# Peiyannn/MM-PDE

Hardware: AMD Instinct MI355X
Metric: MM-PDE rollout node-updates/sec, cylinder 2521-node mesh, 1/2/4/8 GPUs (higher is better)
Workload: dtype f32 (every GNN GEMM fp32-emulated by the fp16x3 split with fp32 accumulate: edge message_net_2, node update_net_1/_2 and message_net_1 projections, embedding; DMM, ItpNet, res_cut, kNN and heads exact fp32); 1 GPU; cy-mmpde; trajectories_per_gpu=16, global_trajectories=16, nodes_per_trajectory=2521, neighbors=35, parallelism=trajectory-shard x1 (no data-path collective), rollout=autoregressive (pred -> next input), launch=eager, three HIP streams, stream_priorities=False

## Files before the change

### mm-pde_amd/csrc/layer.hip

```cpp
#include "common.hpp"
#include <type_traits>
#include "f16x3.hpp"
#include "layer.hpp"

namespace {

constexpr int LH = 128;
constexpr int ET = 16;
constexpr int ESL = 4;
constexpr int ERING = 3;
constexpr int EPF = ERING - 1;
constexpr int SLOT4 = 512;
constexpr int NLDA = LH + 4;

__device__ __forceinline__ void tile_schedule(int bid, int G, int ntiles, int &first, int &stride,
                                              int &count) {
    const int x = bid & 7, i = bid >> 3;
    const int q = G >> 3, rem = G & 7;
    const int nW = q + (x < rem ? 1 : 0);
    const int cum = x * q + min(x, rem);
    const int lo = (int)((int64_t)ntiles * cum / G);
    const int hi = (int)((int64_t)ntiles * (cum + nW) / G);
    first = lo + i;
    stride = nW;
// ... 319 lines not shown
                        for (int cc = 0; cc < CT; ++cc) Ssave[cc] = S[cc];
                        pend = cC.j;
                    }
#pragma unroll
                    for (int cc = 0; cc < CT; ++cc) S[cc] = (f32x4){0.0f, 0.0f, 0.0f, 0.0f};
                }
                cC.next(rpt);
                slot = slot == ERING - 1 ? 0 : slot + 1;
            }
            __syncthreads();
        }
        finish_pending();
    }
}

struct NodeArgs {
    const float *h, *mean;
    int64_t n;
    const float *u1, *c1;
    int64_t ld_u1;
    const float *u2, *c2;
    const float *bn_w, *bn_b, *bn_rm, *bn_rv;
    float eps;
    float *h_out;
    const float *w1n, *b1n;
    int64_t ld_w1n;
    float *a_out, *b_out;
    const float *u, *pos;
    mmpde_gnn_scales sc;
    const char *pk, *pkn;
    float *rmx_out;
    int64_t seg_n;
    const int32_t *div_deg = nullptr;
    int div_k = 0;
    EdgeSplit split;
};

constexpr int NLD = 132;
constexpr int RB = 2;
constexpr int ROWS = 16 * RB;
constexpr int NODE_WPE = 4;

__device__ __forceinline__ void prep_item(int idx, int &row, int &part) {
    row = (idx >> 6) * 8 + (idx & 7);
    part = (idx >> 3) & 7;
}

__device__ __forceinline__ void prep_fetch(const float *src, int64_t lds, int64_t row0, int64_t nrows_valid,
                                           bool global, int row, int part, float4 (&x)[4]) {
    const int64_t srow = global ? min(row0 + row, nrows_valid - 1) : row;
    const float *sp = src + srow * lds + 16 * part;
#pragma unroll
    for (int q = 0; q < 4; ++q) x[q] = *(const float4 *)(sp + 4 * q);
}

template <bool F16X3>
__device__ __forceinline__ void prep_finish(float4 (&x)[4], int64_t srow, int row, int part, float4 *img,
                                            int KT, int kofs, float *rs, float *copy, const int32_t *div_deg,
                                            int div_k, const EdgeSplit *split) {
    if (split && split->units > 0) {
        const SideUnits su = side_units(*split, srow);
        for (int64_t w = su.lo; w <= su.hi; ++w) {
            const float *q4 = split->side + ((su.sg * split->units + w) * 16 + (su.q & 15)) * 128 + 16 * part;
#pragma unroll
            for (int q = 0; q < 4; ++q) {
                const float4 y = *(const float4 *)(q4 + 4 * q);
                x[q] = make_float4(x[q].x + y.x, x[q].y + y.y, x[q].z + y.z, x[q].w + y.w);
            }
        }
    }
    if (div_k > 0) {
        const float d = div_deg ? (float)max(div_deg[srow], 1) : (float)div_k;
        div_rows_rn(x, d);
    }
    if (copy) {
#pragma unroll
        for (int q = 0; q < 4; ++q) *(float4 *)(copy + row * NLD + 16 * part + 4 * q) = x[q];
    }
    const int rb = row >> 4, rr = row & 15;
    if (F16X3) {
        float m = 0.0f;
#pragma unroll
        for (int q = 0; q < 4; ++q) m = absmax4(m, x[q]);
        m = absmax_stride8(m);
        const float s = split_scale(m);
        if (part == 0) rs[row] = s;
#pragma unroll
        for (int q = 0; q < 4; ++q) x[q] = make_float4(x[q].x * s, x[q].y * s, x[q].z * s, x[q].w * s);
        const int KS = KT / 32;
        const int ks = (kofs + 16 * part) >> 5;
        const int g0 = 2 * (part & 1);
#pragma unroll
        for (int hh = 0; hh < 2; ++hh) {
            half8 hi, lo;
            split8_rn(x[2 * hh], x[2 * hh + 1], hi, lo);
            float4 *d = img + ((rb * KS + ks) * 2) * 64 + 16 * (g0 + hh) + rr;
            d[0] = *(const float4 *)&hi;
            d[64] = *(const float4 *)&lo;
        }
    } else {
        const int KJ = KT / 16;
        const int j = (kofs >> 4) + part;
#pragma unroll
        for (int q = 0; q < 4; ++q) img[(rb * KJ + j) * 64 + 16 * q + rr] = x[q];
    }
}

template <bool F16X3>
__device__ __forceinline__ void prep(const float *src, int64_t lds, int64_t row0, int64_t nrows_valid,
                                     bool global, float4 *img, int KT, int kofs, float *rs,
                                     float *copy = nullptr, int t0 = -1, int nthr = 512,
                                     const int32_t *div_deg = nullptr, int div_k = 0,
                                     const EdgeSplit *split = nullptr) {
    for (int idx = t0 < 0 ? (int)threadIdx.x : (int)threadIdx.x - t0; idx < ROWS * 8; idx += nthr) {
        int row, part;
        prep_item(idx, row, part);
        float4 x[4];
        prep_fetch(src, lds, row0, nrows_valid, global, row, part, x);
        const int64_t srow = global ? min(row0 + row, nrows_valid - 1) : row;
        prep_finish<F16X3>(x, srow, row, part, img, KT, kofs, rs, copy, div_deg, div_k, split);
    }
}

template <bool F16X3, int NS>
struct BOps {
    half8 h[F16X3 ? NS : 1], l[F16X3 ? NS : 1];
    float4 w[F16X3 ? 1 : NS];
    __device__ __forceinline__ void load(const char *bimg, int KSB, int ct, int sb0,
                                         const float *wrow, int wk0, int lane) {
#pragma unroll
        for (int s = 0; s < NS; ++s) {
            if (F16X3) {
                h[s] = bfrag(bimg, KSB, ct, sb0 + s, 0, lane);
                l[s] = bfrag(bimg, KSB, ct, sb0 + s, 1, lane);
            } else {
                w[s] = *(const float4 *)(wrow + wk0 + 16 * s + 4 * (lane >> 4));
            }
        }
    }
};

template <bool F16X3, int NS>
__device__ __forceinline__ void gemm_tile(f32x4 *acc, const float4 *img, int KT, int s0,
                                          const BOps<F16X3, NS> &B, int lane) {
#pragma unroll
    for (int s = 0; s < NS; ++s) {
#pragma unroll
        for (int rb = 0; rb < RB; ++rb) {
            if (F16X3) {
                const int KS = KT / 32;
                const float4 h4 = img[((rb * KS + s0 + s) * 2) * 64 + lane];
                const float4 l4 = img[((rb * KS + s0 + s) * 2 + 1) * 64 + lane];
                const half8 ah = *(const half8 *)&h4, al = *(const half8 *)&l4;
                acc[rb] = mfma_f16(ah, B.h[s], acc[rb]);
                acc[rb] = mfma_f16(ah, B.l[s], acc[rb]);
                acc[rb] = mfma_f16(al, B.h[s], acc[rb]);
            } else {
                const int KJ = KT / 16;
                const float4 a = img[(rb * KJ + s0 + s) * 64 + lane];
                acc[rb] = mfma16(a.x, B.w[s].x, acc[rb]);
                acc[rb] = mfma16(a.y, B.w[s].y, acc[rb]);
                acc[rb] = mfma16(a.z, B.w[s].z, acc[rb]);
                acc[rb] = mfma16(a.w, B.w[s].w, acc[rb]);
            }
        }
    }
}

constexpr int MAX_TW = 16;

struct RowValues {
    float t = 0.0f, x = 0.0f, y = 0.0f, u[MAX_TW];
    __device__ __forceinline__ void fetch(const mmpde_gnn_scales &sc, const float *pos, const float *uu,
                                          int64_t row, int tw) {
        const float *pr = sc.pos_xy ? pos + row * 2 : pos + row * 3 + 1;
        x = pr[0];
        y = pr[1];
        t = sc.pos_xy ? (sc.t_ptr ? *sc.t_ptr : sc.t) : pr[-1];
#pragma unroll
        for (int c = 0; c < MAX_TW; ++c) u[c] = c < tw ? uu[row * tw + c] : 0.0f;
    }
    __device__ __forceinline__ void store(float (*rowv)[ROWS], const mmpde_gnn_scales &sc, int tid, int tw) const {
        rowv[0][tid] = t * sc.inv_tmax;
        rowv[1][tid] = x * sc.inv_lx;
        rowv[2][tid] = y * sc.inv_ly;
#pragma unroll
        for (int c = 0; c < MAX_TW; ++c)
            if (c < tw) rowv[3 + c][tid] = u[c];
    }
};

struct W1C {
    float du = 0.0f, dx = 0.0f, dy = 0.0f, t = 0.0f, b = 0.0f, isa = 1.0f, isb = 1.0f;
    template <bool F16X3>
    __device__ __forceinline__ void load(const float *w1r, const float *b1, const char *pk, int col,
                                         int tw) {
        du = w1r[256];
        dx = w1r[256 + tw];
        dy = w1r[257 + tw];
        t = w1r[258 + tw];
        b = b1[col];
        if (F16X3) {
            const float *su = (const float *)(pk + kPkW1 + 131072);
            isa = pow2_inv(su[col]);
            isb = pow2_inv(su[128 + col]);
        }
    }
};

template <bool F16X3>
__device__ __forceinline__ void proj_phase(const BOps<F16X3, F16X3 ? 4 : 8> &bA, const float4 *img,
                                           const float *rs, const float *rowv, const W1C &w,
                                           const char *pk, const float *w1r, int tw, int64_t row0,
                                           int64_t n, int64_t seg_n, float *a_out, float *b_out,
                                           float *rmx_out, uint32_t *arrived, int wave, int lane) {
    constexpr int S1 = F16X3 ? 4 : 8;
    const int col = 16 * wave + (lane & 15), g = lane >> 4;
    f32x4 aA[RB], aB[RB];
#pragma unroll
    for (int rb = 0; rb < RB; ++rb) aA[rb] = aB[rb] = (f32x4){0.0f, 0.0f, 0.0f, 0.0f};
    uint32_t amx[RB][4], bmx[RB][4];
#pragma unroll
    for (int rb = 0; rb < RB; ++rb)
#pragma unroll
        for (int q = 0; q < 4; ++q) amx[rb][q] = bmx[rb][q] = 0u;
    const bool full = row0 + ROWS <= n;
    float *ap = a_out + (row0 + 4 * g) * LH + col, *bp = b_out + (row0 + 4 * g) * LH + col;
    auto node_term = [&](int lr) {
        float node = w.du * rowv[3 * ROWS + lr];
        for (int c = 1; c < tw; ++c) node += w1r[256 + c] * rowv[(3 + c) * ROWS + lr];
        return node + w.dx * rowv[ROWS + lr] + w.dy * rowv[2 * ROWS + lr];
    };
    gemm_tile<F16X3, S1>(aA, img, 128, 0, bA, lane);
    {
        BOps<F16X3, S1> bB;
        bB.load(pk + kPkW1, 4, 8 + wave, 0, w1r, 128, lane);
        gemm_tile<F16X3, S1>(aB, img, 128, 0, bB, lane);
#pragma unroll
        for (int rb = 0; rb < RB; ++rb) {
#pragma unroll
            for (int q = 0; q < 4; ++q) {
                const int lr = 16 * rb + 4 * g + q;
                if (full || row0 + lr < n) {
                    float za = aA[rb][q], zb = aB[rb][q];
                    if (F16X3) {
                        const float ir = pow2_inv(rs[lr]);
                        za = za * ir * w.isa;
                        zb = zb * ir * w.isb;
                    }
                    const float node = node_term(lr);
                    const float va = za + node + w.t * rowv[lr] + w.b;
                    const float vb = zb - node;
                    ap[(16 * rb + q) * LH] = va;
                    bp[(16 * rb + q) * LH] = vb;
                    amx[rb][q] = __builtin_bit_cast(uint32_t, fmaxf(fabsf(va), 0.0f));
                    bmx[rb][q] = __builtin_bit_cast(uint32_t, fmaxf(fabsf(vb), 0.0f));
                }
            }
        }
    }
    if (rmx_out) {
        __shared__ uint32_t red[8][ROWS][2];
#pragma unroll
        for (int rb = 0; rb < RB; ++rb) {
#pragma unroll
            for (int q = 0; q < 4; ++q) {
                uint32_t ua = amx[rb][q], ub = bmx[rb][q];
                ua = max(ua, dpp_u<0xB1>(ua));
                ub = max(ub, dpp_u<0xB1>(ub));
                ua = max(ua, dpp_u<0x4E>(ua));
                ub = max(ub, dpp_u<0x4E>(ub));
                ua = max(ua, dpp_u<0x141>(ua));
                ub = max(ub, dpp_u<0x141>(ub));
                ua = max(ua, dpp_u<0x140>(ua));
                ub = max(ub, dpp_u<0x140>(ub));
                if ((lane & 15) == 0) {
                    red[wave][16 * rb + 4 * g + q][0] = ua;
                    red[wave][16 * rb + 4 * g + q][1] = ub;
                }
            }
        }
        asm volatile("s_waitcnt lgkmcnt(0)" ::: "memory");
        uint32_t prev = 0;
        if (lane == 0) prev = __hip_atomic_fetch_add(arrived, 1u, __ATOMIC_RELAXED, __HIP_MEMORY_SCOPE_WORKGROUP);
        prev = __builtin_amdgcn_readfirstlane(prev);
        asm volatile("s_waitcnt lgkmcnt(0)" ::: "memory");
        if (prev == 7) {
            static_assert(2 * ROWS % 64 == 0, "row maxima: whole waves");
#pragma unroll
            for (int l0 = 0; l0 < 2 * ROWS; l0 += 64) {
                const int l = l0 + lane, row = l >> 1, e = l & 1;
                uint32_t m = red[0][row][e];
#pragma unroll
                for (int w2 = 1; w2 < 8; ++w2) m = max(m, red[w2][row][e]);
                const int64_t grow = row0 + row, b0 = row0 + 16 * (row >> 4);
                const bool live = grow < n;
                if (live) rmx_out[2 * grow + e] = __builtin_bit_cast(float, m);
                const bool part1 = grow >= (b0 / seg_n + 1) * seg_n;
                uint32_t mx0 = live && !part1 ? m : 0u, mx1 = live && part1 ? m : 0u;
                uint32_t mn0 = live && !part1 ? m : 0x7f800000u, mn1 = live && part1 ? m : 0x7f800000u;
                auto xmax = [&](uint32_t &v, auto O) {
                    v = max(v, __builtin_bit_cast(uint32_t, xor_lane_f<decltype(O)::value>(__builtin_bit_cast(float, v))));
                };
                auto xmin = [&](uint32_t &v, auto O) {
                    v = min(v, __builtin_bit_cast(uint32_t, xor_lane_f<decltype(O)::value>(__builtin_bit_cast(float, v))));
                };
                using X2 = std::integral_constant<int, 2>;
                using X4 = std::integral_constant<int, 4>;
                using X8 = std::integral_constant<int, 8>;
                using X16 = std::integral_constant<int, 16>;
                xmax(mx0, X2{}); xmax(mx1, X2{}); xmin(mn0, X2{}); xmin(mn1, X2{});
                xmax(mx0, X4{}); xmax(mx1, X4{}); xmin(mn0, X4{}); xmin(mn1, X4{});
                xmax(mx0, X8{}); xmax(mx1, X8{}); xmin(mn0, X8{}); xmin(mn1, X8{});
                xmax(mx0, X16{}); xmax(mx1, X16{}); xmin(mn0, X16{}); xmin(mn1, X16{});
                if ((l & 31) < 2 && b0 < n) {
                    float *rec = rmx_out + row_max_floats(n) + 8 * (b0 / 16);
                    rec[e] = __builtin_bit_cast(float, mx0);
                    rec[2 + e] = __builtin_bit_cast(float, mn0);
                    rec[4 + e] = __builtin_bit_cast(float, mx1);
                    rec[6 + e] = __builtin_bit_cast(float, mn1);
                }
            }
        }
    }
}

#ifdef MMPDE_NODE_STAMPS
__device__ uint64_t *g_node_stamps;
#define NODE_STAMP(i)                                                                       \
    do {                                                                                   \
        if (threadIdx.x == 0) g_node_stamps[(int64_t)blockIdx.x * 8 + (i)] = __builtin_amdgcn_s_memrealtime(); \
    } while (0)
#else
#define NODE_STAMP(i) \
    do {              \
    } while (0)
#endif

template <bool NEXT, bool F16X3>
__global__ __launch_bounds__(512, NODE_WPE) void gnn_node_kernel(NodeArgs p) {
    NODE_STAMP(0);
    __shared__ float4 img[RB * 16 * 64];
    __shared__ float stage[ROWS * NLD];
    __shared__ float hres[ROWS * NLD];
    __shared__ float rs[4][ROWS];
    __shared__ float rowv[3 + MAX_TW][ROWS];
    __shared__ uint32_t rng_arrived;
    const int tid = threadIdx.x, wave = tid >> 6, lane = tid & 63;
    const int r = lane & 15, g = lane >> 4;
    const int col = 16 * wave + r;
    if (tid == 0) rng_arrived = 0;
    const int tw = p.sc.tw > 1 ? p.sc.tw : 1;
    constexpr int S1 = F16X3 ? 4 : 8;
    const float *wu1 = p.u1 + (int64_t)col * p.ld_u1, *wu2 = p.u2 + (int64_t)col * LH;
    const int64_t row0 = (int64_t)blockIdx.x * ROWS;
    RowValues rv;
    if (tid < ROWS) rv.fetch(p.sc, p.pos, p.u, min(row0 + tid, p.n - 1), tw);
    const float u1_wt = wu1[256], u1_b = p.c1[col];
    const float u1_is = F16X3 ? pow2_inv(((const float *)(p.pk + kPkU1 + 131072))[col]) : 1.0f;
    const float u2_b = p.c2[col];
    BnAffine bn;
    bn.set(p.bn_rm[col], p.bn_rv[col], p.bn_w[col], p.bn_b[col], p.eps);
    const float u2_is = F16X3 ? pow2_inv(((const float *)(p.pk + kPkU2 + 65536))[col]) : 1.0f;
    const float *w1r = NEXT ? p.w1n + (int64_t)col * p.ld_w1n : nullptr;
    W1C w1c;
    if (NEXT) w1c.load<F16X3>(w1r, p.b1n, p.pkn, col, tw);
    BOps<F16X3, S1> bH, bM, bU2;
    bH.load(p.pk + kPkU1, 8, wave, 0, wu1, 0, lane);
    if (tid < ROWS) rv.store(rowv, p.sc, tid, tw);

    NODE_STAMP(1);
    if (tid < 256) prep<F16X3>(p.h, LH, row0, p.n, true, img, 256, 0, rs[0], hres, 0, 256);
    else prep<F16X3>(p.mean, LH, row0, p.n, true, img, 256, 128, rs[1], nullptr, 256, 256, p.div_deg,
                     p.div_k, &p.split);
    __syncthreads();
    NODE_STAMP(2);

    {
        f32x4 aH[RB], aM[RB];
#pragma unroll
        for (int rb = 0; rb < RB; ++rb) aH[rb] = aM[rb] = (f32x4){0.0f, 0.0f, 0.0f, 0.0f};
        gemm_tile<F16X3, S1>(aH, img, 256, 0, bH, lane);
        bM.load(p.pk + kPkU1, 8, wave, S1, wu1, 128, lane);
        gemm_tile<F16X3, S1>(F16X3 ? aM : aH, img, 256, S1, bM, lane);
        bU2.load(p.pk + kPkU2, 4, wave, 0, wu2, 0, lane);
#pragma unroll
        for (int rb = 0; rb < RB; ++rb) {
#pragma unroll
            for (int q = 0; q < 4; ++q) {
                const int lr = 16 * rb + 4 * g + q;
                float v = aH[rb][q];
                if (F16X3) v = v * pow2_inv(rs[0][lr]) * u1_is + aM[rb][q] * pow2_inv(rs[1][lr]) * u1_is;
                stage[lr * NLD + col] = fmaxf(v + u1_wt * rowv[0][lr] + u1_b, 0.0f);
            }
        }
    }
    NODE_STAMP(3);
    __syncthreads();
    prep<F16X3>(stage, NLD, 0, ROWS, false, img, 128, 0, rs[2]);
    __syncthreads();
    NODE_STAMP(4);

    BOps<F16X3, S1> bA;
    {
        f32x4 acc[RB];
#pragma unroll
        for (int rb = 0; rb < RB; ++rb) acc[rb] = (f32x4){0.0f, 0.0f, 0.0f, 0.0f};
        gemm_tile<F16X3, S1>(acc, img, 128, 0, bU2, lane);
        if (NEXT) bA.load(p.pkn + kPkW1, 4, wave, 0, w1r, 0, lane);
        const bool full = row0 + ROWS <= p.n;
        float *hp = p.h_out + (row0 + 4 * g) * LH + col;
#pragma unroll
        for (int rb = 0; rb < RB; ++rb) {
#pragma unroll
            for (int q = 0; q < 4; ++q) {
                const int lr = 16 * rb + 4 * g + q;
                float z = acc[rb][q];
                if (F16X3) z = z * pow2_inv(rs[2][lr]) * u2_is;
                const float x = hres[lr * NLD + col] + fmaxf(z + u2_b, 0.0f);
                const float y = bn(x);
                if (full || row0 + lr < p.n) hp[(16 * rb + q) * LH] = y;
                if (NEXT) stage[lr * NLD + col] = y;
            }
        }
    }
    NODE_STAMP(5);
    if constexpr (NEXT) {
        __syncthreads();
        prep<F16X3>(stage, NLD, 0, ROWS, false, img, 128, 0, rs[3]);
        __syncthreads();
        NODE_STAMP(6);
        proj_phase<F16X3>(bA, img, rs[3], &rowv[0][0], w1c, p.pkn, w1r, tw, row0, p.n, p.seg_n,
                              p.a_out, p.b_out, p.rmx_out, &rng_arrived, wave, lane);
    }
    NODE_STAMP(7);
}

struct EmbedArgs {
    const float *u, *pos;
    int64_t n;
    mmpde_gnn_scales sc;
    mmpde_gnn_embed_params e;
    float *h_out;
    const float *w1, *b1;
    int64_t ld_w1;
    float *a_out, *b_out;
    const char *pk;
    float *rmx_out;
    int64_t seg_n;
};

template <bool F16X3>
__global__ __launch_bounds__(512, NODE_WPE) void gnn_embed_kernel(EmbedArgs p) {
    constexpr int S1 = F16X3 ? 4 : 8;
    __shared__ float4 img[RB * 8 * 64];
    __shared__ float stage[ROWS * NLD];
    __shared__ float rs[ROWS];
    __shared__ uint32_t rng_arrived;
    __shared__ float rsz[ROWS];
    __shared__ float rowv[3 + MAX_TW][ROWS];
    const int tid = threadIdx.x, wave = tid >> 6, lane = tid & 63;
    const int g = lane >> 4;
    const int64_t row0 = (int64_t)blockIdx.x * ROWS;
    const int col = 16 * wave + (lane & 15);
    const int tw = p.sc.tw > 1 ? p.sc.tw : 1;
    if (tid == 0) rng_arrived = 0;
    RowValues rv;
    if (tid < ROWS) rv.fetch(p.sc, p.pos, p.u, min(row0 + tid, p.n - 1), tw);
    const mmpde_gnn_embed_params &e = p.e;
    BOps<false, 8> b3;
    BOps<true, 4> b3h;
    float w3_is = 1.0f;
    if (F16X3) {
        const float *wr = e.w3 + (int64_t)col * LH;
        float4 w[8];
#pragma unroll
        for (int s = 0; s < 4; ++s) {
            w[2 * s] = *(const float4 *)(wr + 32 * s + 8 * g);
            w[2 * s + 1] = *(const float4 *)(wr + 32 * s + 8 * g + 4);
        }
        float m = 0.0f;
#pragma unroll
        for (int i = 0; i < 8; ++i) m = absmax4(m, w[i]);
        m = fmaxf(m, __shfl_xor(m, 16, 64));
        m = fmaxf(m, __shfl_xor(m, 32, 64));
        const float sw = split_scale(m);
        w3_is = pow2_inv(sw);
#pragma unroll
        for (int i = 0; i < 8; ++i) w[i] = make_float4(w[i].x * sw, w[i].y * sw, w[i].z * sw, w[i].w * sw);
#pragma unroll
        for (int s = 0; s < 4; ++s) split8_rn(w[2 * s], w[2 * s + 1], b3h.h[s], b3h.l[s]);
    } else {
        b3.load(nullptr, 0, 0, 0, e.w3 + (int64_t)col * LH, 0, lane);
    }
    const float h_b = e.b3[col];
    BnAffine bn4;
    bn4.set(e.bn4_rm[col], e.bn4_rv[col], e.bn4_w[col], e.bn4_b[col], e.eps);
    const float *w1r = p.w1 + (int64_t)col * p.ld_w1;
    W1C w1c;
    w1c.load<F16X3>(w1r, p.b1, p.pk, col, tw);
    const int c = tid & 127;
    const float *zwr = e.w0 + (int64_t)c * (tw + 3);
    const float zw0 = zwr[0], zw1 = zwr[tw], zw2 = zwr[tw + 1], zw3 = zwr[tw + 2];
    const float zb = e.b0[c];
    BnAffine bn1;
    bn1.set(e.bn1_rm[c], e.bn1_rv[c], e.bn1_w[c], e.bn1_b[c], e.eps);
    if (tid < ROWS) rv.store(rowv, p.sc, tid, tw);
    __syncthreads();
    for (int row = tid >> 7; row < ROWS; row += 4) {
        float v = zb + zw0 * rowv[3][row];
        for (int ch = 1; ch < tw; ++ch) v += zwr[ch] * rowv[3 + ch][row];
        v = v + zw1 * rowv[1][row] + zw2 * rowv[2][row] + zw3 * rowv[0][row];
        stage[row * NLD + c] = fmaxf(bn1(v), 0.0f);
    }
    __syncthreads();
    prep<F16X3>(stage, NLD, 0, ROWS, false, img, 128, 0, rsz);
    __syncthreads();
    BOps<F16X3, S1> bA;
    {
        f32x4 acc[RB];
#pragma unroll
        for (int rb = 0; rb < RB; ++rb) acc[rb] = (f32x4){0.0f, 0.0f, 0.0f, 0.0f};
        if (F16X3) {
            gemm_tile<true, 4>(acc, img, 128, 0, b3h, lane);
#pragma unroll
            for (int rb = 0; rb < RB; ++rb)
#pragma unroll
                for (int q = 0; q < 4; ++q) acc[rb][q] *= pow2_inv(rsz[16 * rb + 4 * g + q]) * w3_is;
        } else {
            gemm_tile<false, 8>(acc, img, 128, 0, b3, lane);
        }
        bA.load(p.pk + kPkW1, 4, wave, 0, w1r, 0, lane);
        const bool full = row0 + ROWS <= p.n;
        float *hp = p.h_out + (row0 + 4 * g) * LH + col;
#pragma unroll
        for (int rb = 0; rb < RB; ++rb) {
#pragma unroll
            for (int q = 0; q < 4; ++q) {
                const int lr = 16 * rb + 4 * g + q;
                const float y = bn4(acc[rb][q] + h_b);
                if (full || row0 + lr < p.n) hp[(16 * rb + q) * LH] = y;
                stage[lr * NLD + col] = y;
            }
        }
    }
    __syncthreads();
    prep<F16X3>(stage, NLD, 0, ROWS, false, img, 128, 0, rs);
    __syncthreads();
    proj_phase<F16X3>(bA, img, rs, &rowv[0][0], w1c, p.pk, w1r, tw, row0, p.n, p.seg_n,
                          p.a_out, p.b_out, p.rmx_out, &rng_arrived, wave, lane);
}

inline bool al16(const void *q) { return ((uintptr_t)q & 15u) == 0; }

int device_cus() {
    int dev = 0, cus = 0;
    if (hipGetDevice(&dev) != hipSuccess) return 256;
    if (hipDeviceGetAttribute(&cus, hipDeviceAttributeMultiprocessorCount, dev) != hipSuccess || cus < 1)
        return 256;
    return cus;
}

}

int launch_edge_stage(const float *a, const float *b, const int32_t *nbr, const int32_t *deg,
                      int64_t n, int k, int64_t seg_n, const mmpde_gnn_layer_params *p, const char *pk,
                      const float *rmx, float *mean, float *side, int64_t side_cap,
                      EdgeSplit *split, hipStream_t st, uint32_t *relu_mask, bool rng) {
    if (split) *split = EdgeSplit{};
    MMPDE_REQUIRE(!relu_mask || (!pk && al16(relu_mask)));
    MMPDE_REQUIRE(a && b && nbr && p && mean && n > 0 && k > 0 && n <= (int64_t)INT32_MAX);
    MMPDE_REQUIRE(al16(a) && al16(b) && al16(p->msg2_w) && al16(mean));
    MMPDE_REQUIRE(!pk || (rmx && al16(pk) && al16(rmx)));
    const int64_t ntiles = (n + ET - 1) / ET;
    MMPDE_REQUIRE(ntiles * ((k + ESL - 1) / ESL) < (int64_t)INT32_MAX);
    const int cus = device_cus();
    if (pk)
        return launch_edge_wave(a, b, nbr, deg, n, k, seg_n, p->msg2_b, pk, rmx, rng, mean, side, side_cap, cus,
                                split, st);
    EdgeArgs e{a, b, nbr, n, k, (int)ntiles, p->msg2_w, p->msg2_b, nullptr, nullptr, mean, deg, relu_mask};
    const int grid = ntiles < cus ? (int)ntiles : cus;
    if (deg) hipLaunchKernelGGL((gnn_edge_kernel<false, true>), dim3(grid), dim3(768), 0, st, e);
    else hipLaunchKernelGGL((gnn_edge_kernel<false, false>), dim3(grid), dim3(768), 0, st, e);
    MMPDE_RET_LAUNCH();
    return MMPDE_OK;
}

__global__ __launch_bounds__(256) void row_max_kernel(const float *__restrict__ a, const float *__restrict__ b,
                                                      int64_t n, float *__restrict__ rmx) {
    const int64_t row = (int64_t)blockIdx.x * 8 + (threadIdx.x >> 5);
    const int c4 = threadIdx.x & 31;
    const int64_t rr = min(row, n - 1);
    float ma = absmax4(0.0f, *(const float4 *)(a + rr * LH + 4 * c4));
    float mb = absmax4(0.0f, *(const float4 *)(b + rr * LH + 4 * c4));
#pragma unroll
    for (int o = 16; o >= 1; o >>= 1) {
        ma = fmaxf(ma, __shfl_xor(ma, o, 32));
        mb = fmaxf(mb, __shfl_xor(mb, o, 32));
    }
    if (c4 == 0 && row < n) *(float2 *)(rmx + 2 * row) = make_float2(ma, mb);
}

__global__ __launch_bounds__(256) void row_scale_kernel(const float *__restrict__ rmx, const int32_t *__restrict__ nbr,
                                                        const int32_t *__restrict__ deg, int64_t n, int k,
                                                        float *__restrict__ rsc) {
    const int64_t row = (int64_t)blockIdx.x * 256 + threadIdx.x;
    if (row >= n) return;
    const int kk = deg ? max(min(deg[row], k), 1) : k;
    const float mb = nbr_bmax<36>(rmx, nbr + row * k, kk, (uint32_t)(n - 1));
    rsc[row] = row_split_scale(rmx[2 * row] + mb);
}

__global__ __launch_bounds__(256) void edge_finish_kernel(float *__restrict__ mean, EdgeSplit sp,
                                                          const int32_t *__restrict__ deg, int64_t n) {
    const int64_t row = (int64_t)blockIdx.x * 32 + (threadIdx.x >> 3);
    const int part = threadIdx.x & 7;
    if (row >= n) return;
    float *mp = mean + row * LH + 16 * part;
    float4 x[4];
#pragma unroll
    for (int q = 0; q < 4; ++q) x[q] = *(const float4 *)(mp + 4 * q);
    const SideUnits su = side_units(sp, row);
    for (int64_t w = su.lo; w <= su.hi; ++w) {
        const float *q4 = sp.side + ((su.sg * sp.units + w) * 16 + (su.q & 15)) * LH + 16 * part;
#pragma unroll
        for (int q = 0; q < 4; ++q) {
            const float4 y = *(const float4 *)(q4 + 4 * q);
            x[q] = make_float4(x[q].x + y.x, x[q].y + y.y, x[q].z + y.z, x[q].w + y.w);
        }
    }
    div_rows_rn(x, deg ? (float)max(deg[row], 1) : (float)sp.k);
#pragma unroll
    for (int q = 0; q < 4; ++q) *(float4 *)(mp + 4 * q) = x[q];
}

int64_t edge_mean_f16x3_ws_bytes(int64_t n) {
    const int64_t tail = ((n + 15) / 16) * 16 * LH;
    return kLayerPack + (row_max_floats(n) + tail) * 4;
}

int launch_edge_mean_f16x3(const float *a, const float *b, const int32_t *nbr, const int32_t *deg, int64_t n,
                           int k, const float *w2, const float *b2, float *mean, uint32_t *relu_mask, void *ws,
                           hipStream_t st) {
    MMPDE_REQUIRE(a && b && nbr && w2 && b2 && mean && ws && n > 0 && k > 0 && n <= (int64_t)INT32_MAX);
    MMPDE_REQUIRE(al16(a) && al16(b) && al16(w2) && al16(mean) && al16(ws));
    MMPDE_REQUIRE(!relu_mask || al16(relu_mask));
    const int64_t ntiles = (n + ET - 1) / ET;
    MMPDE_REQUIRE(ntiles * ((k + ESL - 1) / ESL) < (int64_t)INT32_MAX);
    char *pk = (char *)ws;
    float *rmx = (float *)(pk + kLayerPack);
    float *rsc = rmx + row_max_floats(n);
    PackSrc src{};
    src.w[0] = w2;
    src.ld[0] = LH;
    hipLaunchKernelGGL(pack_f16x3_kernel<128>, dim3(128, 1), dim3(128), 0, st, src, 0, kPkW2, (int64_t)128, pk);
    MMPDE_RET_LAUNCH();
    hipLaunchKernelGGL(row_max_kernel, dim3((unsigned)ceil_div(n, 8)), dim3(256), 0, st, a, b, n, rmx);
    MMPDE_RET_LAUNCH();
    const int cus = device_cus();
    if (!relu_mask) {
        float *side = rsc;
        EdgeSplit split;
        const int rc = launch_edge_wave(a, b, nbr, deg, n, k, n, b2, pk, rmx, false, mean, side, ntiles, cus,
                                        &split, st);
        if (rc) return rc;
        MMPDE_REQUIRE(split.units > 0);
        hipLaunchKernelGGL(edge_finish_kernel, dim3((unsigned)ceil_div(n, 32)), dim3(256), 0, st, mean, split,
                           deg, n);
        MMPDE_RET_LAUNCH();
        return MMPDE_OK;
    }
    hipLaunchKernelGGL(row_scale_kernel, dim3((unsigned)ceil_div(n, 256)), dim3(256), 0, st, rmx, nbr, deg, n, k,
                       rsc);
    MMPDE_RET_LAUNCH();
    EdgeArgs e{a, b, nbr, n, k, (int)ntiles, w2, b2, pk, rsc, mean, deg, relu_mask};
    const int grid = ntiles < cus ? (int)ntiles : cus;
    if (deg) hipLaunchKernelGGL((gnn_edge_kernel<true, true>), dim3(grid), dim3(768), 0, st, e);
    else hipLaunchKernelGGL((gnn_edge_kernel<true, false>), dim3(grid), dim3(768), 0, st, e);
    MMPDE_RET_LAUNCH();
    return MMPDE_OK;
}

int launch_node_stage(const float *h, const float *mean, const EdgeSplit *split, const int32_t *deg,
                      const float *u, const float *pos, int64_t n, int64_t seg_n, mmpde_gnn_scales sc,
                      const mmpde_gnn_layer_params *p, const mmpde_gnn_layer_params *next,
                      const char *pk, const char *pkn, float *rmx_out, float *h_out, float *a_out,
                      float *b_out, hipStream_t st) {
    const bool sums = split && split->units > 0;
    MMPDE_REQUIRE(!sums || (split->side && split->S > 0 && split->k > 0 && split->seg_n > 0 &&
                            n % split->seg_n == 0));
    MMPDE_REQUIRE(!rmx_out || al16(rmx_out));
    MMPDE_REQUIRE(h && mean && u && pos && p && h_out && n > 0);
    MMPDE_REQUIRE(al16(h) && al16(mean) && al16(h_out));
    MMPDE_REQUIRE(p->upd1_ld >= 257 && (p->upd1_ld & 3) == 0 && al16(p->upd1_w) && al16(p->upd2_w));
    MMPDE_REQUIRE(!pk || (al16(pk) && (!next || pkn)));
    NodeArgs a{h, mean, n, p->upd1_w, p->upd1_b, p->upd1_ld, p->upd2_w, p->upd2_b, p->bn_w, p->bn_b,
               p->bn_rm, p->bn_rv, p->eps, h_out, nullptr, nullptr, 0, a_out, b_out, u, pos, sc,
               pk, pkn, rmx_out, effective_seg(n, seg_n), sums ? deg : nullptr,
               sums ? split->k : 0};
    if (sums) a.split = *split;
    if (next) {
        MMPDE_REQUIRE(a_out && b_out && next->msg1_ld >= 260 && (next->msg1_ld & 3) == 0 &&
                      al16(next->msg1_w));
        a.w1n = next->msg1_w;
        a.b1n = next->msg1_b;
        a.ld_w1n = next->msg1_ld;
    }
    const int64_t tiles = ceil_div(n, ROWS);
    MMPDE_REQUIRE(tiles < (int64_t)INT32_MAX);
    const dim3 grid((unsigned)tiles);
    const bool f16 = pk != nullptr;
#define MMPDE_NODE(NX, F16) hipLaunchKernelGGL((gnn_node_kernel<NX, F16>), grid, dim3(512), 0, st, a)
    if (next && f16) MMPDE_NODE(true, true);
    else if (next) MMPDE_NODE(true, false);
    else if (f16) MMPDE_NODE(false, true);
    else MMPDE_NODE(false, false);
#undef MMPDE_NODE
    MMPDE_RET_LAUNCH();
    return MMPDE_OK;
}

int launch_embed_stage(const float *u, const float *pos, int64_t n, int64_t seg_n, mmpde_gnn_scales sc,
                       const mmpde_gnn_embed_params *e, const mmpde_gnn_layer_params *l0,
                       const char *pk0, float *rmx_out, float *h_out, float *a_out,
                       float *b_out, hipStream_t st) {
    MMPDE_REQUIRE(u && pos && e && l0 && h_out && a_out && b_out && n > 0);
    MMPDE_REQUIRE(al16(e->w3) && al16(h_out) && al16(a_out) && al16(b_out));
    MMPDE_REQUIRE(l0->msg1_ld >= 260 && (l0->msg1_ld & 3) == 0 && al16(l0->msg1_w));
    MMPDE_REQUIRE(!pk0 || (al16(pk0) && rmx_out && al16(rmx_out)));
    const EmbedArgs a{u, pos, n, sc, *e, h_out, l0->msg1_w, l0->msg1_b, l0->msg1_ld, a_out,
                      b_out, pk0, rmx_out, effective_seg(n, seg_n)};
    const int64_t tiles = ceil_div(n, ROWS);
    MMPDE_REQUIRE(tiles < (int64_t)INT32_MAX);
    const dim3 grid((unsigned)tiles);
    if (pk0) hipLaunchKernelGGL(gnn_embed_kernel<true>, grid, dim3(512), 0, st, a);
    else hipLaunchKernelGGL(gnn_embed_kernel<false>, grid, dim3(512), 0, st, a);
    MMPDE_RET_LAUNCH();
    return MMPDE_OK;
}
```

Before: 21.01 million node-updates/s.

## Transpose MFMA operands so each lane owns four columns and stores float4

Swaps the A/B operands of every MFMA in gemm_tile, so each lane's accumulator holds four adjacent output columns of one row instead of four rows of one column. Epilogues in the node, embed and projection phases now load per-column constants (bias, BN affine, split scales, msg1 node weights) as float4 from shared-memory tables and write results with 16-byte vector stores to global memory and LDS. The row-max reduction is rewritten around the new lane mapping. This adds shared-memory column tables (aliased onto red/hres in the node kernel, extra LDS in embed) and new 16-byte alignment requirements on bias pointers.

Result: no change. 21.06 million node-updates/s (median of 4 runs) (+0.2%).

```diff
diff --git a/mm-pde_amd/csrc/layer.hip b/mm-pde_amd/csrc/layer.hip
--- a/mm-pde_amd/csrc/layer.hip
+++ b/mm-pde_amd/csrc/layer.hip
@@ -495,16 +495,16 @@
                 const float4 h4 = img[((rb * KS + s0 + s) * 2) * 64 + lane];
                 const float4 l4 = img[((rb * KS + s0 + s) * 2 + 1) * 64 + lane];
                 const half8 ah = *(const half8 *)&h4, al = *(const half8 *)&l4;
-                acc[rb] = mfma_f16(ah, B.h[s], acc[rb]);
-                acc[rb] = mfma_f16(ah, B.l[s], acc[rb]);
-                acc[rb] = mfma_f16(al, B.h[s], acc[rb]);
+                acc[rb] = mfma_f16(B.h[s], ah, acc[rb]);
+                acc[rb] = mfma_f16(B.l[s], ah, acc[rb]);
+                acc[rb] = mfma_f16(B.h[s], al, acc[rb]);
             } else {
                 const int KJ = KT / 16;
                 const float4 a = img[(rb * KJ + s0 + s) * 64 + lane];
-                acc[rb] = mfma16(a.x, B.w[s].x, acc[rb]);
-                acc[rb] = mfma16(a.y, B.w[s].y, acc[rb]);
-                acc[rb] = mfma16(a.z, B.w[s].z, acc[rb]);
-                acc[rb] = mfma16(a.w, B.w[s].w, acc[rb]);
+                acc[rb] = mfma16(B.w[s].x, a.x, acc[rb]);
+                acc[rb] = mfma16(B.w[s].y, a.y, acc[rb]);
+                acc[rb] = mfma16(B.w[s].z, a.z, acc[rb]);
+                acc[rb] = mfma16(B.w[s].w, a.w, acc[rb]);
             }
         }
     }
@@ -533,95 +533,110 @@
     }
 };
 
-struct W1C {
-    float du = 0.0f, dx = 0.0f, dy = 0.0f, t = 0.0f, b = 0.0f, isa = 1.0f, isb = 1.0f;
-    template <bool F16X3>
-    __device__ __forceinline__ void load(const float *w1r, const float *b1, const char *pk, int col,
-                                         int tw) {
-        du = w1r[256];
-        dx = w1r[256 + tw];
-        dy = w1r[257 + tw];
+__device__ __forceinline__ void f4arr(const float4 &v, float (&a)[4]) {
+    a[0] = v.x, a[1] = v.y, a[2] = v.z, a[3] = v.w;
+}
+
+constexpr int W1T_PLANES = 3 + MAX_TW;
+struct W1Cols {
+    float t = 0.0f, x = 0.0f, y = 0.0f, u0 = 0.0f;
+    __device__ __forceinline__ void fetch(const float *w1r, int tw) {
+        u0 = w1r[256];
+        x = w1r[256 + tw];
+        y = w1r[257 + tw];
         t = w1r[258 + tw];
-        b = b1[col];
-        if (F16X3) {
-            const float *su = (const float *)(pk + kPkW1 + 131072);
-            isa = pow2_inv(su[col]);
-            isb = pow2_inv(su[128 + col]);
-        }
+    }
+    __device__ __forceinline__ void store(float *w1t, const float *w1r, int col, int tw) const {
+        w1t[col] = t;
+        w1t[LH + col] = x;
+        w1t[2 * LH + col] = y;
+        w1t[3 * LH + col] = u0;
+        for (int c = 1; c < tw; ++c) w1t[(3 + c) * LH + col] = w1r[256 + c];
     }
 };
 
 template <bool F16X3>
 __device__ __forceinline__ void proj_phase(const BOps<F16X3, F16X3 ? 4 : 8> &bA, const float4 *img,
-                                           const float *rs, const float *rowv, const W1C &w,
-                                           const char *pk, const float *w1r, int tw, int64_t row0,
-                                           int64_t n, int64_t seg_n, float *a_out, float *b_out,
-                                           float *rmx_out, uint32_t *arrived, int wave, int lane) {
+                                           const float *rs, const float *rowv, const float *w1t,
+                                           const float *b1, const char *pk, const float *w1r, int tw,
+                                           int64_t row0, int64_t n, int64_t seg_n, float *a_out,
+                                           float *b_out, float *rmx_out, uint32_t (*red)[ROWS][2],
+                                           uint32_t *arrived, int wave, int lane) {
     constexpr int S1 = F16X3 ? 4 : 8;
-    const int col = 16 * wave + (lane & 15), g = lane >> 4;
+    const int r = lane & 15, g = lane >> 4;
+    const int c4 = 16 * wave + 4 * g;
     f32x4 aA[RB], aB[RB];
 #pragma unroll
     for (int rb = 0; rb < RB; ++rb) aA[rb] = aB[rb] = (f32x4){0.0f, 0.0f, 0.0f, 0.0f};
-    uint32_t amx[RB][4], bmx[RB][4];
-#pragma unroll
-    for (int rb = 0; rb < RB; ++rb)
-#pragma unroll
-        for (int q = 0; q < 4; ++q) amx[rb][q] = bmx[rb][q] = 0u;
+    uint32_t amx[RB], bmx[RB];
     const bool full = row0 + ROWS <= n;
-    float *ap = a_out + (row0 + 4 * g) * LH + col, *bp = b_out + (row0 + 4 * g) * LH + col;
-    auto node_term = [&](int lr) {
-        float node = w.du * rowv[3 * ROWS + lr];
-        for (int c = 1; c < tw; ++c) node += w1r[256 + c] * rowv[(3 + c) * ROWS + lr];
-        return node + w.dx * rowv[ROWS + lr] + w.dy * rowv[2 * ROWS + lr];
-    };
     gemm_tile<F16X3, S1>(aA, img, 128, 0, bA, lane);
     {
         BOps<F16X3, S1> bB;
         bB.load(pk + kPkW1, 4, 8 + wave, 0, w1r, 128, lane);
+        float wb[4], isa[4] = {1.0f, 1.0f, 1.0f, 1.0f}, isb[4] = {1.0f, 1.0f, 1.0f, 1.0f};
+        f4arr(*(const float4 *)(b1 + c4), wb);
+        if (F16X3) {
+            const float *su = (const float *)(pk + kPkW1 + 131072);
+            float sa[4], sb[4];
+            f4arr(*(const float4 *)(su + c4), sa);
+            f4arr(*(const float4 *)(su + 128 + c4), sb);
+#pragma unroll
+            for (int q = 0; q < 4; ++q) isa[q] = pow2_inv(sa[q]), isb[q] = pow2_inv(sb[q]);
+        }
         gemm_tile<F16X3, S1>(aB, img, 128, 0, bB, lane);
+        float wt[4], wx[4], wy[4], wu[4];
+        f4arr(*(const float4 *)(w1t + c4), wt);
+        f4arr(*(const float4 *)(w1t + LH + c4), wx);
+        f4arr(*(const float4 *)(w1t + 2 * LH + c4), wy);
+        f4arr(*(const float4 *)(w1t + 3 * LH + c4), wu);
 #pragma unroll
         for (int rb = 0; rb < RB; ++rb) {
+            const int lr = 16 * rb + r;
+            amx[rb] = bmx[rb] = 0u;
+            const float ir = F16X3 ? pow2_inv(rs[lr]) : 1.0f;
+            const float tr = rowv[lr], xr = rowv[ROWS + lr], yr = rowv[2 * ROWS + lr];
+            float node[4];
+            {
+                const float u0 = rowv[3 * ROWS + lr];
+#pragma unroll
+                for (int q = 0; q < 4; ++q) node[q] = wu[q] * u0;
+            }
+            for (int c = 1; c < tw; ++c) {
+                float wc[4];
+                f4arr(*(const float4 *)(w1t + (3 + c) * LH + c4), wc);
+                const float uc = rowv[(3 + c) * ROWS + lr];
+#pragma unroll
+                for (int q = 0; q < 4; ++q) node[q] += wc[q] * uc;
+            }
+            float va[4], vb[4];
 #pragma unroll
             for (int q = 0; q < 4; ++q) {
-                const int lr = 16 * rb + 4 * g + q;
-                if (full || row0 + lr < n) {
-                    float za = aA[rb][q], zb = aB[rb][q];
-                    if (F16X3) {
-                        const float ir = pow2_inv(rs[lr]);
-                        za = za * ir * w.isa;
-                        zb = zb * ir * w.isb;
-                    }
-                    const float node = node_term(lr);
-                    const float va = za + node + w.t * rowv[lr] + w.b;
-                    const float vb = zb - node;
-                    ap[(16 * rb + q) * LH] = va;
-                    bp[(16 * rb + q) * LH] = vb;
-                    amx[rb][q] = __builtin_bit_cast(uint32_t, fmaxf(fabsf(va), 0.0f));
-                    bmx[rb][q] = __builtin_bit_cast(uint32_t, fmaxf(fabsf(vb), 0.0f));
+                float za = aA[rb][q], zb = aB[rb][q];
+                if (F16X3) {
+                    za = za * ir * isa[q];
+                    zb = zb * ir * isb[q];
+                }
+                const float nd = node[q] + wx[q] * xr + wy[q] * yr;
+                va[q] = za + nd + wt[q] * tr + wb[q];
+                vb[q] = zb - nd;
+            }
+            if (full || row0 + lr < n) {
+                *(float4 *)(a_out + (row0 + lr) * LH + c4) = make_float4(va[0], va[1], va[2], va[3]);
+                *(float4 *)(b_out + (row0 + lr) * LH + c4) = make_float4(vb[0], vb[1], vb[2], vb[3]);
+#pragma unroll
+                for (int q = 0; q < 4; ++q) {
+                    amx[rb] = max(amx[rb], __builtin_bit_cast(uint32_t, fmaxf(fabsf(va[q]), 0.0f)));
+                    bmx[rb] = max(bmx[rb], __builtin_bit_cast(uint32_t, fmaxf(fabsf(vb[q]), 0.0f)));
                 }
             }
         }
     }
     if (rmx_out) {
-        __shared__ uint32_t red[8][ROWS][2];
 #pragma unroll
         for (int rb = 0; rb < RB; ++rb) {
-#pragma unroll
-            for (int q = 0; q < 4; ++q) {
-                uint32_t ua = amx[rb][q], ub = bmx[rb][q];
-                ua = max(ua, dpp_u<0xB1>(ua));
-                ub = max(ub, dpp_u<0xB1>(ub));
-                ua = max(ua, dpp_u<0x4E>(ua));
-                ub = max(ub, dpp_u<0x4E>(ub));
-                ua = max(ua, dpp_u<0x141>(ua));
-                ub = max(ub, dpp_u<0x141>(ub));
-                ua = max(ua, dpp_u<0x140>(ua));
-                ub = max(ub, dpp_u<0x140>(ub));
-                if ((lane & 15) == 0) {
-                    red[wave][16 * rb + 4 * g + q][0] = ua;
-                    red[wave][16 * rb + 4 * g + q][1] = ub;
-                }
-            }
+            const uint32_t ua = umax_rows32(umax_rows16(amx[rb])), ub = umax_rows32(umax_rows16(bmx[rb]));
+            if (g == 0) *(uint2 *)&red[wave][16 * rb + r][0] = make_uint2(ua, ub);
         }
         asm volatile("s_waitcnt lgkmcnt(0)" ::: "memory");
         uint32_t prev = 0;
@@ -684,14 +699,19 @@
 __global__ __launch_bounds__(512, NODE_WPE) void gnn_node_kernel(NodeArgs p) {
     NODE_STAMP(0);
     __shared__ float4 img[RB * 16 * 64];
-    __shared__ float stage[ROWS * NLD];
-    __shared__ float hres[ROWS * NLD];
+    __shared__ __attribute__((aligned(16))) float stage[ROWS * NLD];
+    __shared__ __attribute__((aligned(16))) float hres[ROWS * NLD];
     __shared__ float rs[4][ROWS];
     __shared__ float rowv[3 + MAX_TW][ROWS];
     __shared__ uint32_t rng_arrived;
+    __shared__ __attribute__((aligned(16))) uint32_t red[8][ROWS][2];
+    static_assert(sizeof(red) >= 3 * LH * sizeof(float) && sizeof(hres) >= W1T_PLANES * LH * sizeof(float),
+                  "column tables alias red / hres");
+    float *bnt = (float *)&red[0][0][0], *w1t = hres;
     const int tid = threadIdx.x, wave = tid >> 6, lane = tid & 63;
     const int r = lane & 15, g = lane >> 4;
     const int col = 16 * wave + r;
+    const int c4 = 16 * wave + 4 * g;
     if (tid == 0) rng_arrived = 0;
     const int tw = p.sc.tw > 1 ? p.sc.tw : 1;
     constexpr int S1 = F16X3 ? 4 : 8;
@@ -699,15 +719,17 @@
     const int64_t row0 = (int64_t)blockIdx.x * ROWS;
     RowValues rv;
     if (tid < ROWS) rv.fetch(p.sc, p.pos, p.u, min(row0 + tid, p.n - 1), tw);
-    const float u1_wt = wu1[256], u1_b = p.c1[col];
-    const float u1_is = F16X3 ? pow2_inv(((const float *)(p.pk + kPkU1 + 131072))[col]) : 1.0f;
-    const float u2_b = p.c2[col];
-    BnAffine bn;
-    bn.set(p.bn_rm[col], p.bn_rv[col], p.bn_w[col], p.bn_b[col], p.eps);
-    const float u2_is = F16X3 ? pow2_inv(((const float *)(p.pk + kPkU2 + 65536))[col]) : 1.0f;
     const float *w1r = NEXT ? p.w1n + (int64_t)col * p.ld_w1n : nullptr;
-    W1C w1c;
-    if (NEXT) w1c.load<F16X3>(w1r, p.b1n, p.pkn, col, tw);
+    const float *w1c_row = NEXT ? p.w1n + (int64_t)(tid & (LH - 1)) * p.ld_w1n : nullptr;
+    W1Cols w1c;
+    if (tid < LH) {
+        if (NEXT) w1c.fetch(w1c_row, tw);
+        BnAffine bn;
+        bn.set(p.bn_rm[tid], p.bn_rv[tid], p.bn_w[tid], p.bn_b[tid], p.eps);
+        bnt[tid] = bn.a;
+        bnt[LH + tid] = bn.c;
+        bnt[2 * LH + tid] = p.u1[(int64_t)tid * p.ld_u1 + 256];
+    }
     BOps<F16X3, S1> bH, bM, bU2;
     bH.load(p.pk + kPkU1, 8, wave, 0, wu1, 0, lane);
     if (tid < ROWS) rv.store(rowv, p.sc, tid, tw);
@@ -723,19 +745,32 @@
         f32x4 aH[RB], aM[RB];
 #pragma unroll
         for (int rb = 0; rb < RB; ++rb) aH[rb] = aM[rb] = (f32x4){0.0f, 0.0f, 0.0f, 0.0f};
+        float u1_wt[4], u1_b[4], u1_is[4] = {1.0f, 1.0f, 1.0f, 1.0f};
+        f4arr(*(const float4 *)(p.c1 + c4), u1_b);
+        if (F16X3) {
+            float s[4];
+            f4arr(*(const float4 *)((const float *)(p.pk + kPkU1 + 131072) + c4), s);
+#pragma unroll
+            for (int q = 0; q < 4; ++q) u1_is[q] = pow2_inv(s[q]);
+        }
         gemm_tile<F16X3, S1>(aH, img, 256, 0, bH, lane);
         bM.load(p.pk + kPkU1, 8, wave, S1, wu1, 128, lane);
         gemm_tile<F16X3, S1>(F16X3 ? aM : aH, img, 256, S1, bM, lane);
         bU2.load(p.pk + kPkU2, 4, wave, 0, wu2, 0, lane);
+        f4arr(*(const float4 *)(bnt + 2 * LH + c4), u1_wt);
 #pragma unroll
         for (int rb = 0; rb < RB; ++rb) {
+            const int lr = 16 * rb + r;
+            const float ih = F16X3 ? pow2_inv(rs[0][lr]) : 1.0f, im = F16X3 ? pow2_inv(rs[1][lr]) : 1.0f;
+            const float tr = rowv[0][lr];
+            float o[4];
 #pragma unroll
             for (int q = 0; q < 4; ++q) {
-                const int lr = 16 * rb + 4 * g + q;
                 float v = aH[rb][q];
-                if (F16X3) v = v * pow2_inv(rs[0][lr]) * u1_is + aM[rb][q] * pow2_inv(rs[1][lr]) * u1_is;
-                stage[lr * NLD + col] = fmaxf(v + u1_wt * rowv[0][lr] + u1_b, 0.0f);
-            }
+                if (F16X3) v = v * ih * u1_is[q] + aM[rb][q] * im * u1_is[q];
+                o[q] = fmaxf(v + u1_wt[q] * tr + u1_b[q], 0.0f);
+            }
+            *(float4 *)&stage[lr * NLD + c4] = make_float4(o[0], o[1], o[2], o[3]);
         }
     }
     NODE_STAMP(3);
@@ -749,32 +784,47 @@
         f32x4 acc[RB];
 #pragma unroll
         for (int rb = 0; rb < RB; ++rb) acc[rb] = (f32x4){0.0f, 0.0f, 0.0f, 0.0f};
+        float u2_b[4], u2_is[4] = {1.0f, 1.0f, 1.0f, 1.0f};
+        f4arr(*(const float4 *)(p.c2 + c4), u2_b);
+        if (F16X3) {
+            float s[4];
+            f4arr(*(const float4 *)((const float *)(p.pk + kPkU2 + 65536) + c4), s);
+#pragma unroll
+            for (int q = 0; q < 4; ++q) u2_is[q] = pow2_inv(s[q]);
+        }
         gemm_tile<F16X3, S1>(acc, img, 128, 0, bU2, lane);
         if (NEXT) bA.load(p.pkn + kPkW1, 4, wave, 0, w1r, 0, lane);
         const bool full = row0 + ROWS <= p.n;
-        float *hp = p.h_out + (row0 + 4 * g) * LH + col;
+        float bna[4], bnc[4];
+        f4arr(*(const float4 *)(bnt + c4), bna);
+        f4arr(*(const float4 *)(bnt + LH + c4), bnc);
 #pragma unroll
         for (int rb = 0; rb < RB; ++rb) {
+            const int lr = 16 * rb + r;
+            const float iv = F16X3 ? pow2_inv(rs[2][lr]) : 1.0f;
+            float hr[4], y[4];
+            f4arr(*(const float4 *)&hres[lr * NLD + c4], hr);
 #pragma unroll
             for (int q = 0; q < 4; ++q) {
-                const int lr = 16 * rb + 4 * g + q;
                 float z = acc[rb][q];
-                if (F16X3) z = z * pow2_inv(rs[2][lr]) * u2_is;
-                const float x = hres[lr * NLD + col] + fmaxf(z + u2_b, 0.0f);
-                const float y = bn(x);
-                if (full || row0 + lr < p.n) hp[(16 * rb + q) * LH] = y;
-                if (NEXT) stage[lr * NLD + col] = y;
-            }
+                if (F16X3) z = z * iv * u2_is[q];
+                const float x = hr[q] + fmaxf(z + u2_b[q], 0.0f);
+                y[q] = fmaf(x, bna[q], bnc[q]);
+            }
+            const float4 y4 = make_float4(y[0], y[1], y[2], y[3]);
+            if (full || row0 + lr < p.n) *(float4 *)(p.h_out + (row0 + lr) * LH + c4) = y4;
+            if (NEXT) *(float4 *)&stage[lr * NLD + c4] = y4;
         }
     }
     NODE_STAMP(5);
     if constexpr (NEXT) {
         __syncthreads();
+        if (tid < LH) w1c.store(w1t, w1c_row, tid, tw);
         prep<F16X3>(stage, NLD, 0, ROWS, false, img, 128, 0, rs[3]);
         __syncthreads();
         NODE_STAMP(6);
-        proj_phase<F16X3>(bA, img, rs[3], &rowv[0][0], w1c, p.pkn, w1r, tw, row0, p.n, p.seg_n,
-                              p.a_out, p.b_out, p.rmx_out, &rng_arrived, wave, lane);
+        proj_phase<F16X3>(bA, img, rs[3], &rowv[0][0], w1t, p.b1n, p.pkn, w1r, tw, row0, p.n, p.seg_n,
+                          p.a_out, p.b_out, p.rmx_out, red, &rng_arrived, wave, lane);
     }
     NODE_STAMP(7);
 }
@@ -797,15 +847,19 @@
 __global__ __launch_bounds__(512, NODE_WPE) void gnn_embed_kernel(EmbedArgs p) {
     constexpr int S1 = F16X3 ? 4 : 8;
     __shared__ float4 img[RB * 8 * 64];
-    __shared__ float stage[ROWS * NLD];
+    __shared__ __attribute__((aligned(16))) float stage[ROWS * NLD];
     __shared__ float rs[ROWS];
     __shared__ uint32_t rng_arrived;
     __shared__ float rsz[ROWS];
     __shared__ float rowv[3 + MAX_TW][ROWS];
+    __shared__ __attribute__((aligned(16))) float colt[3][LH];
+    __shared__ __attribute__((aligned(16))) float w1t[W1T_PLANES * LH];
+    __shared__ __attribute__((aligned(16))) uint32_t red[8][ROWS][2];
     const int tid = threadIdx.x, wave = tid >> 6, lane = tid & 63;
-    const int g = lane >> 4;
+    const int r = lane & 15, g = lane >> 4;
     const int64_t row0 = (int64_t)blockIdx.x * ROWS;
-    const int col = 16 * wave + (lane & 15);
+    const int col = 16 * wave + r;
+    const int c4 = 16 * wave + 4 * g;
     const int tw = p.sc.tw > 1 ? p.sc.tw : 1;
     if (tid == 0) rng_arrived = 0;
     RowValues rv;
@@ -829,6 +883,7 @@
         m = fmaxf(m, __shfl_xor(m, 32, 64));
         const float sw = split_scale(m);
         w3_is = pow2_inv(sw);
+        if (g == 0) colt[2][col] = w3_is;
 #pragma unroll
         for (int i = 0; i < 8; ++i) w[i] = make_float4(w[i].x * sw, w[i].y * sw, w[i].z * sw, w[i].w * sw);
 #pragma unroll
@@ -836,12 +891,17 @@
     } else {
         b3.load(nullptr, 0, 0, 0, e.w3 + (int64_t)col * LH, 0, lane);
     }
-    const float h_b = e.b3[col];
-    BnAffine bn4;
-    bn4.set(e.bn4_rm[col], e.bn4_rv[col], e.bn4_w[col], e.bn4_b[col], e.eps);
     const float *w1r = p.w1 + (int64_t)col * p.ld_w1;
-    W1C w1c;
-    w1c.load<F16X3>(w1r, p.b1, p.pk, col, tw);
+    if (tid < LH) {
+        BnAffine bn4;
+        bn4.set(e.bn4_rm[tid], e.bn4_rv[tid], e.bn4_w[tid], e.bn4_b[tid], e.eps);
+        colt[0][tid] = bn4.a;
+        colt[1][tid] = bn4.c;
+        const float *w1c_row = p.w1 + (int64_t)tid * p.ld_w1;
+        W1Cols w1c;
+        w1c.fetch(w1c_row, tw);
+        w1c.store(w1t, w1c_row, tid, tw);
+    }
     const int c = tid & 127;
     const float *zwr = e.w0 + (int64_t)c * (tw + 3);
     const float zw0 = zwr[0], zw1 = zwr[tw], zw2 = zwr[tw + 1], zw3 = zwr[tw + 2];
@@ -864,34 +924,41 @@
         f32x4 acc[RB];
 #pragma unroll
         for (int rb = 0; rb < RB; ++rb) acc[rb] = (f32x4){0.0f, 0.0f, 0.0f, 0.0f};
+        float h_b[4], bna[4], bnc[4];
+        f4arr(*(const float4 *)(e.b3 + c4), h_b);
+        f4arr(*(const float4 *)(&colt[0][c4]), bna);
+        f4arr(*(const float4 *)(&colt[1][c4]), bnc);
         if (F16X3) {
             gemm_tile<true, 4>(acc, img, 128, 0, b3h, lane);
-#pragma unroll
-            for (int rb = 0; rb < RB; ++rb)
-#pragma unroll
-                for (int q = 0; q < 4; ++q) acc[rb][q] *= pow2_inv(rsz[16 * rb + 4 * g + q]) * w3_is;
+            float is3[4];
+            f4arr(*(const float4 *)(&colt[2][c4]), is3);
+#pragma unroll
+            for (int rb = 0; rb < RB; ++rb) {
+                const float iz = pow2_inv(rsz[16 * rb + r]);
+#pragma unroll
+                for (int q = 0; q < 4; ++q) acc[rb][q] *= iz * is3[q];
+            }
         } else {
             gemm_tile<false, 8>(acc, img, 128, 0, b3, lane);
         }
         bA.load(p.pk + kPkW1, 4, wave, 0, w1r, 0, lane);
         const bool full = row0 + ROWS <= p.n;
-        float *hp = p.h_out + (row0 + 4 * g) * LH + col;
 #pragma unroll
         for (int rb = 0; rb < RB; ++rb) {
-#pragma unroll
-            for (int q = 0; q < 4; ++q) {
-                const int lr = 16 * rb + 4 * g + q;
-                const float y = bn4(acc[rb][q] + h_b);
-                if (full || row0 + lr < p.n) hp[(16 * rb + q) * LH] = y;
-                stage[lr * NLD + col] = y;
-            }
+            const int lr = 16 * rb + r;
+            float y[4];
+#pragma unroll
+            for (int q = 0; q < 4; ++q) y[q] = fmaf(acc[rb][q] + h_b[q], bna[q], bnc[q]);
+            const float4 y4 = make_float4(y[0], y[1], y[2], y[3]);
+            if (full || row0 + lr < p.n) *(float4 *)(p.h_out + (row0 + lr) * LH + c4) = y4;
+            *(float4 *)&stage[lr * NLD + c4] = y4;
         }
     }
     __syncthreads();
     prep<F16X3>(stage, NLD, 0, ROWS, false, img, 128, 0, rs);
     __syncthreads();
-    proj_phase<F16X3>(bA, img, rs, &rowv[0][0], w1c, p.pk, w1r, tw, row0, p.n, p.seg_n,
-                          p.a_out, p.b_out, p.rmx_out, &rng_arrived, wave, lane);
+    proj_phase<F16X3>(bA, img, rs, &rowv[0][0], w1t, p.b1, p.pk, w1r, tw, row0, p.n, p.seg_n, p.a_out,
+                      p.b_out, p.rmx_out, red, &rng_arrived, wave, lane);
 }
 
 inline bool al16(const void *q) { return ((uintptr_t)q & 15u) == 0; }
@@ -1037,6 +1104,8 @@
     MMPDE_REQUIRE(al16(h) && al16(mean) && al16(h_out));
     MMPDE_REQUIRE(p->upd1_ld >= 257 && (p->upd1_ld & 3) == 0 && al16(p->upd1_w) && al16(p->upd2_w));
     MMPDE_REQUIRE(!pk || (al16(pk) && (!next || pkn)));
+    MMPDE_REQUIRE(p->upd1_b && p->upd2_b && al16(p->upd1_b) && al16(p->upd2_b));
+    MMPDE_REQUIRE(!next || (next->msg1_b && al16(next->msg1_b)));
     NodeArgs a{h, mean, n, p->upd1_w, p->upd1_b, p->upd1_ld, p->upd2_w, p->upd2_b, p->bn_w, p->bn_b,
                p->bn_rm, p->bn_rv, p->eps, h_out, nullptr, nullptr, 0, a_out, b_out, u, pos, sc,
                pk, pkn, rmx_out, effective_seg(n, seg_n), sums ? deg : nullptr,
@@ -1071,6 +1140,7 @@
     MMPDE_REQUIRE(al16(e->w3) && al16(h_out) && al16(a_out) && al16(b_out));
     MMPDE_REQUIRE(l0->msg1_ld >= 260 && (l0->msg1_ld & 3) == 0 && al16(l0->msg1_w));
     MMPDE_REQUIRE(!pk0 || (al16(pk0) && rmx_out && al16(rmx_out)));
+    MMPDE_REQUIRE(e->b3 && l0->msg1_b && al16(e->b3) && al16(l0->msg1_b));
     const EmbedArgs a{u, pos, n, sc, *e, h_out, l0->msg1_w, l0->msg1_b, l0->msg1_ld, a_out,
                       b_out, pk0, rmx_out, effective_seg(n, seg_n)};
     const int64_t tiles = ceil_div(n, ROWS);
```
